# DarylFernandes99/custom-yolo-implmentation

Measured on AMD Instinct MI355X. Metric: images/sec (640x640 bf16), higher is better.
Workload: dtype bf16; 1 GPU; preset s (width 32..512, depth 1) 640x640 train step (fwd+DFL/QFL loss+bwd+grad sync+AdamW), COCO-80 synthetic, 32 img/GPU; global_batch=32, parallelism=dp1, hip_graph=True, optimizer_in_graph=True, deterministic_mode=False

## Files before the change

custom-yolo-implmentation_amd/csrc/conv_generic.hip:

```cpp
#include "conv_host.h"

namespace {

template <typename T, int V, bool ACC>
__global__ void k_conv_generic(ConvGeom g, const T* __restrict__ src, const T* __restrict__ wm,
                               const float* __restrict__ bias, T* __restrict__ dst) {
    long total = (long)g.N * g.Hg * g.Wg * g.Cd;
    for (long i = blockIdx.x * (long)blockDim.x + threadIdx.x; i < total; i += (long)gridDim.x * blockDim.x) {
        int cd = (int)(i % g.Cd);
        long q = i / g.Cd;
        int b = (int)(q % g.Wg);
        long t2 = q / g.Wg;
        int a = (int)(t2 % g.Hg);
        long n = t2 / g.Hg;
        float acc = bias ? bias[cd] : 0.f;
        const T* wrow = wm + (long)cd * g.Kpad;
        for (int t = 0; t < g.ntaps; ++t) {
            int hs = a * g.sstride + g.dh[t], ws = b * g.sstride + g.dw[t];
            if (hs < 0 || hs >= g.Hs || ws < 0 || ws >= g.Ws) continue;
            const T* sp = src + ((n * g.Hs + hs) * g.Ws + ws) * (long)g.lds;
            const T* wp = wrow + t * g.Cs;
            for (int c = 0; c < g.Cs; c += V) {
                float xs[V], wv[V];
                load_pack<T, V>(sp + c, xs);
// ... 218 lines not shown
                                               (const T*)src, (const T*)wm, bias, (T*)dst);
            else hipLaunchKernelGGL((k_conv_generic<T, V, false>), dim3(grid_for(total)), dim3(256), 0, st, g,
                                    (const T*)src, (const T*)wm, bias, (T*)dst);
        } else {
            if (accumulate) hipLaunchKernelGGL((k_conv_generic<T, 1, true>), dim3(grid_for(total)), dim3(256), 0, st, g,
                                               (const T*)src, (const T*)wm, bias, (T*)dst);
            else hipLaunchKernelGGL((k_conv_generic<T, 1, false>), dim3(grid_for(total)), dim3(256), 0, st, g,
                                    (const T*)src, (const T*)wm, bias, (T*)dst);
        }
    });
    return YOLO_LAUNCH_CHECK();
}

}

int valu_conv_launch(const ConvGeom& g, const void* src, const void* wm, const float* bias, void* dst, int accumulate, int dtype,
                     hipStream_t st) {
    int rc = launch_generic(g, src, wm, bias, dst, accumulate, dtype, st);
    if (rc == YOLO_OK && accumulate && g.acc2 != nullptr)
        rc = yolo_copy_channels(g.acc2, g.ld2, dst, g.ldd, (long)g.N * g.Hd * g.Wd, g.Cd, 1, dtype, st);
    if (rc == YOLO_OK && g.stats)
        rc = yolo_bn_stats_acc(dst, g.ldd, (long)g.N * g.Hd * g.Wd, g.Cd, dtype, g.stats, st);
    return rc;
}

extern "C" {

int yolo_conv_kpad(int O, int I, int k, int stride, int mode, int cls) {
    int dh[9], dw[9], kh[9], kw[9];
    int nt = conv_taps(mode, k, stride, cls, dh, dw, kh, kw);
    return round_up32(nt * (mode == 0 ? I : O));
}

long yolo_conv_dgrad_wbuf_elems(int O, int I, int k, int stride) {
    if (stride == 1) return (long)I * yolo_conv_kpad(O, I, k, 1, 1, 0);
    long s = 0;
    for (int c = 0; c < 4; ++c) s += (long)I * yolo_conv_kpad(O, I, k, 2, 1, c);
    return s;
}

int yolo_conv_pack_weights(const void* w_oihw, int w_dtype, int O, int I, int k, int stride, int mode, void* out,
                           int out_dtype, hipStream_t st) {
    if (!conv_supported(k, stride)) return YOLO_ERR_ARG;
    int ncls = (mode == 1 && stride == 2) ? 4 : 1;
    long off = 0;
    for (int c = 0; c < ncls; ++c) {
        TapIdx taps;
        int dh[9], dw[9];
        taps.n = conv_taps(mode, k, stride, c, dh, dw, taps.kh, taps.kw);
        int Kpad = round_up32(taps.n * (mode == 0 ? I : O));
        long total = (long)(mode == 0 ? O : I) * Kpad;
#define PACK_LAUNCH(P)                                                                                               \
    YOLO_DISPATCH_T(out_dtype, hipLaunchKernelGGL((k_pack_weights<P, T>), dim3(grid_for(total)), dim3(256), 0, st,   \
                                                  (const P*)w_oihw, O, I, k, mode, taps, (T*)out + off, Kpad))
        switch (w_dtype) {
            case YOLO_F32:  PACK_LAUNCH(float); break;
            case YOLO_BF16: PACK_LAUNCH(bf16_t); break;
            case YOLO_F16:  PACK_LAUNCH(f16_t); break;
            default: return YOLO_ERR_DTYPE;
        }
#undef PACK_LAUNCH
        off += total;
    }
    return YOLO_LAUNCH_CHECK();
}

int yolo_conv_unpack_wgrad(const float* dwp, int O, int I, int k, void* dw_oihw, int dw_dtype, hipStream_t st) {
    int Kpad = round_up32(k * k * I);
    long total = (long)O * I * k * k;
    switch (dw_dtype) {
        case YOLO_F32:  hipLaunchKernelGGL((k_unpack_wgrad<float>), dim3(grid_for(total)), dim3(256), 0, st, dwp, O, I, k, Kpad, (float*)dw_oihw); break;
        case YOLO_BF16: hipLaunchKernelGGL((k_unpack_wgrad<bf16_t>), dim3(grid_for(total)), dim3(256), 0, st, dwp, O, I, k, Kpad, (bf16_t*)dw_oihw); break;
        case YOLO_F16:  hipLaunchKernelGGL((k_unpack_wgrad<f16_t>), dim3(grid_for(total)), dim3(256), 0, st, dwp, O, I, k, Kpad, (f16_t*)dw_oihw); break;
        default: return YOLO_ERR_DTYPE;
    }
    return YOLO_LAUNCH_CHECK();
}

long yolo_conv2d_wgrad_plan(int N, int H, int W, int Cin, int OH, int OW, int Cout, int k, int stride, int dtype) {
    if (!conv_supported(k, stride)) return -1;
    static const long long dummy[2] = {0, 0};
    if (!mfma_wgrad_eligible(Cin, Cout, Cin, Cout, dtype, dummy, dummy)) return 0;
    return mfma_wgrad2_plan(round_up32(k * k * Cin), N, H, W, Cin, OH, OW, Cout, k);
}

static int wgrad_path(const void* x, int ldx, const void* dy, int ldy, int N, int H, int W, int Cin, int OH, int OW,
                      int Cout, int dtype, int algo) {
    if (algo != 1 && mfma_wgrad_eligible(Cin, Cout, ldx, ldy, dtype, x, dy)) {
        const bool big = (long)N * H * W * ldx + (long)(W + 1) * ldx >= (1L << 30) || (long)N * OH * OW * ldy >= (1L << 30);
        return (algo == 3 || big || (long)N * OH * OW == 0) ? 3 : 2;
    }
    return 1;
}

long yolo_conv2d_wgrad_ws_elems(const void* x, int ldx, const void* dy, int ldy, int N, int H, int W, int Cin, int OH,
                                int OW, int Cout, int k, int stride, int dtype, int algo) {
    if (!conv_supported(k, stride)) return 0;
    const int Kpad = round_up32(k * k * Cin);
    if (wgrad_path(x, ldx, dy, ldy, N, H, W, Cin, OH, OW, Cout, dtype, algo) == 2)
        return mfma_wgrad2_ws_elems(Kpad, N, H, W, Cin, OH, OW, Cout, k);
    return (long)Cout * Kpad;
}

int yolo_conv2d_wgrad(const void* x, int ldx, const void* dy, int ldy, float* ws, void* dw_oihw, int dw_dtype, int N,
                      int H, int W, int Cin, int OH, int OW, int Cout, int k, int stride, int dtype, int algo,
                      hipStream_t st) {
    if (!conv_supported(k, stride)) return YOLO_ERR_ARG;
    const int K = k * k * Cin, Kpad = round_up32(K);
    const int path = wgrad_path(x, ldx, dy, ldy, N, H, W, Cin, OH, OW, Cout, dtype, algo);
    if (path == 2)
        return mfma_wgrad2_launch(x, ldx, dy, ldy, ws, dw_oihw, dw_dtype, Kpad, N, H, W, Cin, OH, OW, Cout, k, stride, dtype, st);
    if (algo == 2) return YOLO_ERR_ARG;
    float* dwp = ws;
    int rc = yolo_zero_async(dwp, (size_t)Cout * Kpad * sizeof(float), st);
    if (rc) return rc;
    if (path == 3) {
        rc = mfma_wgrad_launch(x, ldx, dy, ldy, dwp, Kpad, N, H, W, Cin, OH, OW, Cout, k, stride, dtype, st);
    } else if (dtype == YOLO_F32 && f32_wgrad_eligible(x, ldx, dy, ldy, Cin, Cout)) {
        rc = f32_wgrad_launch((const float*)x, ldx, (const float*)dy, ldy, dwp, Kpad, N, H, W, Cin, OH, OW, Cout, k, stride, st);
    } else {
        long nrows = (long)N * OH;
        long elems = (long)Cout * K;
        int gx = (int)((elems + 255) / 256);
        long want_slabs = 4096 / (gx > 0 ? gx : 1);
        if (want_slabs < 1) want_slabs = 1;
        if (want_slabs > nrows) want_slabs = nrows;
        if (want_slabs < 1) want_slabs = 1;
        int rps = (int)((nrows + want_slabs - 1) / want_slabs);
        if (rps < 1) rps = 1;
        int gy = (int)((nrows + rps - 1) / rps);
        if (gy > 0)
            YOLO_DISPATCH_T(dtype, hipLaunchKernelGGL((k_wgrad_generic<T>), dim3(gx, gy), dim3(256), 0, st, (const T*)x, ldx,
                                                      (const T*)dy, ldy, dwp, Kpad, N, H, W, Cin, OH, OW, Cout, k, stride, rps));
        rc = YOLO_LAUNCH_CHECK();
    }
    if (rc) return rc;
    return yolo_conv_unpack_wgrad(dwp, Cout, Cin, k, dw_oihw, dw_dtype, st);
}

}

static dim3 dw_grid(int nrows, int cv) {
    int tpr = cv < 256 ? cv : 256;
    return dim3((unsigned)(nrows < 4096 ? nrows : 4096), (unsigned)ceil_div(cv, tpr));
}

template <bool FLIP>
static int dw_launch(const void* x, int ldx, const float* w, void* y, int ldy, int N, int H, int W, int C, int dtype,
                     int accumulate, hipStream_t st) {
    const int fast = dw16_launch(FLIP, x, ldx, w, y, ldy, N, H, W, C, dtype, accumulate, nullptr, st);
    if (fast >= 0) return fast;
    YOLO_DISPATCH_T(dtype, {
        if (vecok<T>(x, ldx, C) && vecok<T>(y, ldy, C)) {
            constexpr int V = vec_of<T>::N;
            hipLaunchKernelGGL((k_dw3x3<T, V, FLIP>), dw_grid(N * H, C / V), dim3(256), 0, st, (const T*)x, ldx, w, (T*)y,
                               ldy, N, H, W, C, accumulate);
        } else {
            hipLaunchKernelGGL((k_dw3x3<T, 1, FLIP>), dw_grid(N * H, C), dim3(256), 0, st, (const T*)x, ldx, w, (T*)y, ldy,
                               N, H, W, C, accumulate);
        }
    });
    return YOLO_LAUNCH_CHECK();
}

extern "C" {

// ... 80 lines not shown
```

custom-yolo-implmentation_amd/csrc/conv_host.h:

```cpp
#pragma once
#include "common.h"
#include "conv_geom.h"

enum ConvKind {
    CONV_NONE = -1,
    CONV_VALU = 0,
    CONV_GATHER = 1,
    CONV_HALO = 2,
    CONV_RING = 3,
    CONV_ROWS = 4,
    CONV_UP2 = 5
};
struct RingTile { int bm, bn, nst, bk; };
struct ConvChoice {
    int kind;
    int joint;
    int variant;
    int bn;
    RingTile ring;
};
ConvChoice conv_select(const ConvGeom* gs, int n, int cls, int dtype, const void* src, const void* wm, const void* dst, int algo);

ConvTune& conv_tune();
int conv_wide_flag();

static inline bool desc_addressable(long elems) { return elems < (1L << 30); }
static inline bool pixels_addressable(long npix) { return npix < (1L << 31); }

int mfma_conv_addressable(const ConvGeom& g, int dtype, const void* src, const void* wm, const void* dst);

int valu_conv_launch(const ConvGeom& g, const void* src, const void* wm, const float* bias, void* dst, int accumulate, int dtype,
                     hipStream_t st);
int mfma_conv_eligible(const ConvGeom& g, int dtype, const void* src, const void* wm, const void* dst);
int mfma_conv_launch(const ConvGeom& g, int bn, const void* src, const void* wm, const float* bias, void* dst, int accumulate,
                     int dtype, hipStream_t st);
int halo_conv_eligible(const ConvGeom& g);
int halo_conv_launch(const ConvGeom& g, int variant, const void* src, const void* wm, const float* bias, void* dst,
                     int accumulate, int dtype, hipStream_t st);
int ring_conv_eligible(const ConvGeom& g, int dtype, const void* src, const void* wm, const void* dst);
int ring_conv_launch(const ConvGeom* gs, int n, const RingTile& t, const long* wm_off, long wm_elems, const void* src,
                     const void* wm, const float* bias, void* dst, int accumulate, int dtype, hipStream_t st);
int rows_conv_eligible(const ConvGeom& g);
int rows_conv_launch(const ConvGeom& g, int variant, const void* src, const void* wm, const float* bias, void* dst, int accumulate,
                     int dtype, hipStream_t st);
int up2_conv_eligible(const ConvGeom* gs, int dtype);
int up2_conv_launch(const ConvGeom* gs, int variant, const long* wm_off, long wm_elems, const void* src, const void* wm, void* dst,
                    int accumulate, int dtype, hipStream_t st);
int f32_conv_eligible(const ConvGeom& g, const void* src, const void* wm, const void* dst);
int f32_conv_launch(const ConvGeom& g, const float* src, const float* wm, const float* bias, float* dst, int accumulate,
                    hipStream_t st);

int f32_wgrad_eligible(const void* x, int ldx, const void* dy, int ldy, int Cin, int Cout);
int f32_wgrad_launch(const float* x, int ldx, const float* dy, int ldy, float* dwp, int Kpad, int N, int H, int W, int Cin,
                     int OH, int OW, int Cout, int k, int stride, hipStream_t st);
int mfma_wgrad_eligible(int Cin, int Cout, int ldx, int ldy, int dtype, const void* x, const void* dy);
int mfma_wgrad_launch(const void* x, int ldx, const void* dy, int ldy, float* dwp, int Kpad, int N, int H, int W,
                      int Cin, int OH, int OW, int Cout, int k, int stride, int dtype, hipStream_t st);
long mfma_wgrad2_plan(int Kpad, int N, int H, int W, int Cin, int OH, int OW, int Cout, int k);
long mfma_wgrad2_ws_elems(int Kpad, int N, int H, int W, int Cin, int OH, int OW, int Cout, int k);
int mfma_wgrad2_launch(const void* x, int ldx, const void* dy, int ldy, float* part, void* dw_oihw, int dw_dtype, int Kpad,
                       int N, int H, int W, int Cin, int OH, int OW, int Cout, int k, int stride, int dtype, hipStream_t st);

struct DwPlan {
    int cvb, ncy;
    int ncol, ncb;
    int wg;
    int hb, nb, grid;
    int hb_wg, nb_wg, grid_wg;
};
DwPlan dw_plan(int N, int H, int W, int C);
int dw_tune_set(int variant);
bool dw_takes_rows(int N, int H, int W, int C, bool wgrad);
int dw16_launch(bool flip, const void* x, int ldx, const float* w, void* y, int ldy, int N, int H, int W, int C, int dtype,
                int accumulate, float* stats, hipStream_t st, const float* bias = nullptr, int act = 0);
int dw16_wgrad_launch(const void* x, int ldx, const void* dy, int ldy, float* partial, int nslab, int* nrows, int N, int H, int W,
                      int C, int dtype, hipStream_t st);

extern "C" int yolo_bn_stats_acc(const void* y, int ldy, long npix, int C, int dtype, float* acc, hipStream_t st);
extern "C" int yolo_copy_channels(const void* src, int ld_src, void* dst, int ld_dst, long npix, int C, int accumulate, int dtype,
                                  hipStream_t st);

static inline bool conv_supported(int k, int stride) { return (k == 1 && stride == 1) || (k == 3 && (stride == 1 || stride == 2)); }
```

custom-yolo-implmentation_amd/csrc/wgrad_mfma.hip:

```cpp
#include <cstdio>
#include <cstdlib>
#include "conv_host.h"

namespace {

typedef __attribute__((ext_vector_type(4))) float f32x4;
typedef __attribute__((ext_vector_type(8))) __bf16 bf16x8;
typedef __attribute__((ext_vector_type(8))) _Float16 f16x8;
typedef __attribute__((ext_vector_type(4))) short s16x4;
typedef __attribute__((ext_vector_type(8))) short s16x8;
typedef unsigned int u32x4 __attribute__((ext_vector_type(4)));

template <typename T> struct mm;
template <> struct mm<bf16_t> {
    typedef bf16x8 frag;
    static __device__ __forceinline__ f32x4 mma(frag a, frag b, f32x4 c) { return __builtin_amdgcn_mfma_f32_16x16x32_bf16(a, b, c, 0, 0, 0); }
};
template <> struct mm<f16_t> {
    typedef f16x8 frag;
    static __device__ __forceinline__ f32x4 mma(frag a, frag b, f32x4 c) { return __builtin_amdgcn_mfma_f32_16x16x32_f16(a, b, c, 0, 0, 0); }
};

constexpr int ldc_of(int t) { return t * 32 + 16; }
constexpr int PWL = 12;

struct WgArgs {
    int N, H, W, Cin, ldx, OH, OW, Cout, ldy, Kpad;
    int pbh, pbw;
    long npatch, per_slab;
    int cot, cit;
    int xcd;
};

__device__ __forceinline__ int xcd_chunk(int bid, int nwg) {
    int q = nwg >> 3, r = nwg & 7, x = bid & 7;
    return (x < r ? x * (q + 1) : r * (q + 1) + (x - r) * q) + (bid >> 3);
}

template <typename T>
__device__ __forceinline__ typename mm<T>::frag tr_frag(const T* p_lo, const T* p_hi) {
    s16x4 lo = __builtin_amdgcn_ds_read_tr16_b64_v4i16((__attribute__((address_space(3))) s16x4*)p_lo);
    s16x4 hi = __builtin_amdgcn_ds_read_tr16_b64_v4i16((__attribute__((address_space(3))) s16x4*)p_hi);
    s16x8 both = __builtin_shufflevector(lo, hi, 0, 1, 2, 3, 4, 5, 6, 7);
    return __builtin_bit_cast(typename mm<T>::frag, both);
}

template <typename T, int KS, int S, int TCO, int TCI, int PF>
__global__ __launch_bounds__(256) void k_wgrad2(WgArgs a, const T* __restrict__ x, const T* __restrict__ dy,
                                                float* __restrict__ dwp) {
    constexpr int PAD = KS / 2;
    constexpr int PH = 3 * S + KS, PW = 7 * S + KS;
    constexpr int LDY = ldc_of(TCO), LDX = ldc_of(TCI);
    constexpr int SUB = ((PH + 1) / 2) * PWL;
    constexpr int XROWS = S == 1 ? PH * PWL : 4 * SUB;
    constexpr int CPY = TCO * 4, CPX = TCI * 4;
    constexpr int YCH = 32 * CPY, YR = (YCH + 255) / 256;
    constexpr int XCH = PH * PW * CPX;
    constexpr int XR = (XCH + 255) / 256;
    constexpr int NT = KS * KS;
    static_assert(PW <= PWL || S == 2, "X patch wider than its LDS image");
    static_assert(S == 1 || (PW + 1) / 2 <= PWL, "parity plane wider than its LDS image");
    __shared__ __attribute__((aligned(16))) T ys[32 * LDY];
    __shared__ __attribute__((aligned(16))) T xs[XROWS * LDX];

    const int tid = threadIdx.x, lane = tid & 63, wave = tid >> 6;
    const int wc = wave >> 1, wi = wave & 1;
    const int unit = a.xcd ? xcd_chunk(blockIdx.x, gridDim.x) : (int)blockIdx.x, ntile = a.cot * a.cit;
    const int slab = unit / ntile, tile = unit - slab * ntile;
    const int bco = (tile % a.cot) * (32 * TCO), bci = (tile / a.cot) * (32 * TCI);
    long p_begin = (long)slab * a.per_slab, p_end = p_begin + a.per_slab;
    if (p_end > a.npatch) p_end = a.npatch;

    f32x4 acc[NT][TCO][TCI];
#pragma unroll
    for (int t = 0; t < NT; ++t)
#pragma unroll
        for (int i = 0; i < TCO; ++i)
#pragma unroll
            for (int j = 0; j < TCI; ++j) acc[t][i][j] = (f32x4){0.f, 0.f, 0.f, 0.f};

    const int xshift = (a.W + 1) * a.ldx;
    const __amdgpu_buffer_rsrc_t rsx = buf_desc(x - xshift, (a.N * a.H * a.W * a.ldx + xshift) * 2);
    const __amdgpu_buffer_rsrc_t rsy = buf_desc(dy, a.N * a.OH * a.OW * a.ldy * 2);
    int yrow[YR], ycol[YR], yvoff[YR], ylds[YR];
#pragma unroll
    for (int r = 0; r < YR; ++r) {
        const int id = tid + 256 * r;
        const int j = id / CPY, ch = (id - j * CPY) * 8;
        yrow[r] = j >> 3;
        ycol[r] = j & 7;
        yvoff[r] = (id < YCH && bco + ch < a.Cout) ? ((yrow[r] * a.OW + ycol[r]) * a.ldy + bco + ch) * 2 : BUF_OOB;
        ylds[r] = id < YCH ? ((j & 3) + 4 * ((j >> 3) & 1) + 8 * ((j >> 2) & 1) + 16 * (j >> 4)) * LDY + ch : -1;
    }
    int xpr[XR], xpc[XR], xvoff[XR], xlds[XR];
#pragma unroll
    for (int r = 0; r < XR; ++r) {
        const int id = tid + 256 * r;
        const int px = id / CPX, ch = (id - px * CPX) * 8;
        xpr[r] = px / PW;
        xpc[r] = px - xpr[r] * PW;
        xvoff[r] = (id < XCH && bci + ch < a.Cin) ? ((xpr[r] * a.W + xpc[r]) * a.ldx + bci + ch) * 2 : BUF_OOB;
        const int row = S == 1 ? xpr[r] * PWL + xpc[r]
                               : ((xpr[r] & 1) * 2 + (xpc[r] & 1)) * SUB + (xpr[r] >> 1) * PWL + (xpc[r] >> 1);
        xlds[r] = id < XCH ? row * LDX + ch : -1;
    }
    int pn, pbh, pbw;
    {
        const int per_img = a.pbh * a.pbw;
        pn = (int)(p_begin / per_img);
        const int rem = (int)(p_begin - (long)pn * per_img);
        pbh = rem / a.pbw;
        pbw = rem - pbh * a.pbw;
    }
    uint4 ry[PF][YR], rx[PF][XR];
    auto gload = [&](uint4 (&ry_)[YR], uint4 (&rx_)[XR], bool live) {
        const int oh0 = pbh * 4, ow0 = pbw * 8;
        const int ih0 = oh0 * S - PAD, iw0 = ow0 * S - PAD;
        const int ysoff = live ? ((pn * a.OH + oh0) * a.OW + ow0) * a.ldy * 2 : 0;
#pragma unroll
        for (int r = 0; r < YR; ++r) {
            const bool ok = live && oh0 + yrow[r] < a.OH && ow0 + ycol[r] < a.OW;
            const u32x4 v = __builtin_amdgcn_raw_buffer_load_b128(rsy, ok ? yvoff[r] : BUF_OOB, ysoff, 0);
            ry_[r] = make_uint4(v.x, v.y, v.z, v.w);
        }
        const int xsoff = live ? (((pn * a.H + ih0) * a.W + iw0) * a.ldx + xshift) * 2 : 0;
#pragma unroll
        for (int r = 0; r < XR; ++r) {
            const bool ok = live && (unsigned)(ih0 + xpr[r]) < (unsigned)a.H && (unsigned)(iw0 + xpc[r]) < (unsigned)a.W;
            const u32x4 v = __builtin_amdgcn_raw_buffer_load_b128(rsx, ok ? xvoff[r] : BUF_OOB, xsoff, 0);
            rx_[r] = make_uint4(v.x, v.y, v.z, v.w);
        }
        if (++pbw == a.pbw) {
            pbw = 0;
            if (++pbh == a.pbh) { pbh = 0; ++pn; }
        }
    };
    auto lstore = [&](const uint4 (&ry_)[YR], const uint4 (&rx_)[XR]) {
#pragma unroll
        for (int r = 0; r < YR; ++r)
            if (ylds[r] >= 0) *reinterpret_cast<uint4*>(ys + ylds[r]) = ry_[r];
#pragma unroll
        for (int r = 0; r < XR; ++r)
            if (xlds[r] >= 0) *reinterpret_cast<uint4*>(xs + xlds[r]) = rx_[r];
    };

    const int g = lane >> 4, i16 = lane & 15, q = i16 >> 2, c4 = 4 * (i16 & 3);
    const T* ya = ys + (q + 4 * (g & 1) + 16 * (g >> 1)) * LDY + wc * TCO * 16 + c4;
    auto compute = [&]() {
        typename mm<T>::frag fa[TCO];
#pragma unroll
        for (int i = 0; i < TCO; ++i) fa[i] = tr_frag<T>(ya + i * 16, ya + i * 16 + 8 * LDY);
#pragma unroll
        for (int kh = 0; kh < KS; ++kh)
#pragma unroll
            for (int kw = 0; kw < KS; ++kw) {
                const int row = S == 1 ? (g + kh) * PWL + q + kw
                                       : ((kh & 1) * 2 + (kw & 1)) * SUB + (g + (kh >> 1)) * PWL + q + (kw >> 1);
                const T* base = xs + row * LDX + wi * TCI * 16 + c4;
#pragma unroll
                for (int j = 0; j < TCI; ++j) {
                    typename mm<T>::frag fb = tr_frag<T>(base + j * 16, base + j * 16 + 4 * LDX);
#pragma unroll
                    for (int i = 0; i < TCO; ++i) acc[kh * KS + kw][i][j] = mm<T>::mma(fa[i], fb, acc[kh * KS + kw][i][j]);
                }
            }
    };
#pragma unroll
    for (int s2 = 0; s2 < PF; ++s2) gload(ry[s2], rx[s2], p_begin + s2 < p_end);
    for (long pi = p_begin; pi < p_end; pi += PF) {
#pragma unroll
        for (int s2 = 0; s2 < PF; ++s2) {
            if (pi + s2 >= p_end) break;
            __syncthreads();
            lstore(ry[s2], rx[s2]);
            __syncthreads();
            gload(ry[s2], rx[s2], pi + s2 + PF < p_end);
            compute();
        }
    }
    float4* part4 = reinterpret_cast<float4*>(dwp) + ((((long)slab * ntile + tile) * 4 + wave) * (NT * TCO * TCI)) * 64 + lane;
#pragma unroll
    for (int t = 0; t < NT; ++t)
#pragma unroll
        for (int i = 0; i < TCO; ++i)
#pragma unroll
            for (int j = 0; j < TCI; ++j) {
                const f32x4 v = acc[t][i][j];
                part4[((t * TCO + i) * TCI + j) * 64] = make_float4(v[0], v[1], v[2], v[3]);
            }
}

template <typename TO, int SL>
__global__ __launch_bounds__(256) void k_wgrad_reduce(const float* __restrict__ part, int nslab, int Cout, int Cin, int NT,
                                                      int tco, int tci, int cot, long groups, TO* __restrict__ dw) {
    constexpr int EL = 256 / SL;
    __shared__ float4 red[SL][EL + 1];
    const int el = threadIdx.x % EL, sl = threadIdx.x / EL;
    const long gi = (long)blockIdx.x * EL + el;
    float4 a = make_float4(0.f, 0.f, 0.f, 0.f);
    if (gi < groups) {
        const float4* p = reinterpret_cast<const float4*>(part) + gi;
#pragma unroll 4
        for (int s2 = sl; s2 < nslab; s2 += SL) {
            const float4 v = p[s2 * groups];
            a.x += v.x; a.y += v.y; a.z += v.z; a.w += v.w;
        }
    }
    if (SL > 1) {
        red[sl][el] = a;
        __syncthreads();
        if (sl != 0) return;
#pragma unroll
        for (int s2 = 1; s2 < SL; ++s2) {
            const float4 v = red[s2][el];
            a.x += v.x; a.y += v.y; a.z += v.z; a.w += v.w;
        }
    }
    if (gi < groups) {
        const int lane = (int)(gi & 63);
        long rest = gi >> 6;
        const int j = (int)(rest % tci); rest /= tci;
        const int i = (int)(rest % tco); rest /= tco;
        const int t = (int)(rest % NT); rest /= NT;
        const int wave = (int)(rest & 3);
        const int tile = (int)(rest >> 2);
        const int co = (tile % cot) * (32 * tco) + ((wave >> 1) * tco + i) * 16 + (lane >> 4) * 4;
        const int ci = (tile / cot) * (32 * tci) + ((wave & 1) * tci + j) * 16 + (lane & 15);
        if (ci < Cin) {
            TO* o = dw + ((long)co * Cin + ci) * NT + t;
            const long rs = (long)Cin * NT;
            if (co < Cout) o[0] = (TO)a.x;
            if (co + 1 < Cout) o[rs] = (TO)a.y;
            if (co + 2 < Cout) o[2 * rs] = (TO)a.z;
            if (co + 3 < Cout) o[3 * rs] = (TO)a.w;
        }
    }
}

struct WgPlan { int to, ti, cot, cit, nslab, pf; long per_slab; };

template <typename TO>
void launch_reduce(const float* part, const WgPlan& p, int Cout, int Cin, int NT, void* dw, hipStream_t st) {
    const long groups = (long)p.cot * p.cit * 4 * NT * p.to * p.ti * 64;
    if (p.nslab >= 32)
        hipLaunchKernelGGL((k_wgrad_reduce<TO, 8>), dim3((unsigned)((groups + 31) / 32)), dim3(256), 0, st, part, p.nslab, Cout, Cin, NT, p.to, p.ti, p.cot, groups, (TO*)dw);
    else if (p.nslab >= 4)
        hipLaunchKernelGGL((k_wgrad_reduce<TO, 4>), dim3((unsigned)((groups + 63) / 64)), dim3(256), 0, st, part, p.nslab, Cout, Cin, NT, p.to, p.ti, p.cot, groups, (TO*)dw);
    else
        hipLaunchKernelGGL((k_wgrad_reduce<TO, 1>), dim3((unsigned)((groups + 255) / 256)), dim3(256), 0, st, part, p.nslab, Cout, Cin, NT, p.to, p.ti, p.cot, groups, (TO*)dw);
}



struct WgTune { int to, ti, blocks, min_per; long all_blocks; int pf; };
WgTune& wg_tune() {
    static WgTune t = [] {
        WgTune v{0, 0, 0, 0, 0, 0};
        if (const char* e = getenv("YOLO_WG_TUNE")) sscanf(e, "%d,%d,%d,%d", &v.to, &v.ti, &v.blocks, &v.min_per);
        if (const char* e2 = getenv("YOLO_WG_BLOCKS")) v.all_blocks = atol(e2);
        if (const char* e3 = getenv("YOLO_WG_PF")) v.pf = atoi(e3);
        return v;
    }();
    return t;
}

WgPlan make_plan(const WgArgs& a, int k) {
    WgPlan p;
    if (k == 1) {
        p.to = a.Cout > 96 ? 4 : a.Cout > 64 ? 3 : a.Cout > 32 ? 2 : 1;
        p.ti = a.Cin > 96 ? 4 : a.Cin > 64 ? 3 : a.Cin > 32 ? 2 : 1;
    } else {
        p.to = a.Cout > 32 ? 2 : 1;
        p.ti = a.Cin > 64 ? 2 : 1;
    }
    const int cot0 = (a.Cout + 32 * p.to - 1) / (32 * p.to), cit0 = (a.Cin + 32 * p.ti - 1) / (32 * p.ti);
    const long data_bytes = ((long)a.N * a.H * a.W * a.Cin + (long)a.N * a.OH * a.OW * a.Cout) * 2;
    long want_blocks;
    const WgTune& tu = wg_tune();
    if (tu.all_blocks > 0) {
        want_blocks = tu.all_blocks;
    } else if (k == 1) {
        if (p.to * p.ti == 1) want_blocks = 2048;
        else want_blocks = (cot0 * cit0 == 1 && data_bytes < (150L << 20)) ? 256 : 512;
    } else {
        want_blocks = p.ti == 1 ? 512 : 256;
    }
    {
        static const double scale = [] { const char* e = getenv("YOLO_WG_SCALE"); return e ? atof(e) : 0.5; }();
        if (scale > 0.0 && tu.all_blocks <= 0 && tu.blocks <= 0) {
            const long tile_bytes = (long)k * k * (32 * p.to) * (32 * p.ti) * 4;
            long cap = (long)(scale * (double)data_bytes / (double)tile_bytes);
            static const long floor_wg = [] { const char* e = getenv("YOLO_WG_FLOOR"); return e ? atol(e) : 128L; }();
            if (cap < floor_wg) cap = floor_wg;
            if (want_blocks > cap) want_blocks = cap;
        }
    }
    long min_per = 2;
    if (tu.to > 0 && (k == 1 || tu.to <= 2)) p.to = tu.to;
    if (tu.ti > 0 && (k == 1 || tu.ti <= 2)) p.ti = tu.ti;
    if (tu.blocks > 0) want_blocks = tu.blocks;
    if (tu.min_per > 0) min_per = tu.min_per;
    p.cot = (a.Cout + 32 * p.to - 1) / (32 * p.to);
    p.cit = (a.Cin + 32 * p.ti - 1) / (32 * p.ti);
    long want = want_blocks / ((long)p.cot * p.cit);
    if (want > a.npatch / min_per) want = a.npatch / min_per;
    if (want < 1) want = 1;
    p.per_slab = (a.npatch + want - 1) / want;
    p.nslab = (int)((a.npatch + p.per_slab - 1) / p.per_slab);
    p.pf = 1;
    if (tu.pf == 1 || tu.pf == 4) p.pf = tu.pf;
    return p;
}

template <typename T, int KS, int S, int TCO, int TCI>
void launch(const WgArgs& a, const WgPlan& p, const void* x, const void* dy, float* part, hipStream_t st) {
    WgArgs b = a;
    b.per_slab = p.per_slab;
    b.cot = p.cot; b.cit = p.cit;
    static const int xcd = [] { const char* e = getenv("YOLO_WG_XCD"); return e ? atoi(e) : 1; }();
    b.xcd = xcd;
    const dim3 grid((unsigned)(p.cot * p.cit * p.nslab));
    if (p.pf == 4)
        hipLaunchKernelGGL((k_wgrad2<T, KS, S, TCO, TCI, 4>), grid, dim3(256), 0, st, b, (const T*)x, (const T*)dy, part);
    else
        hipLaunchKernelGGL((k_wgrad2<T, KS, S, TCO, TCI, 1>), grid, dim3(256), 0, st, b, (const T*)x, (const T*)dy, part);
}

template <typename T, int KS, int S>
void launch_tiles(const WgArgs& a, const WgPlan& p, const void* x, const void* dy, float* part, hipStream_t st) {
#define WG_CASE(TO_, TI_) if (p.to == TO_ && p.ti == TI_) return launch<T, KS, S, TO_, TI_>(a, p, x, dy, part, st)
    if constexpr (KS == 1) {
        WG_CASE(1, 1); WG_CASE(1, 2); WG_CASE(1, 3); WG_CASE(1, 4);
        WG_CASE(2, 1); WG_CASE(2, 2); WG_CASE(2, 3); WG_CASE(2, 4);
        WG_CASE(3, 1); WG_CASE(3, 2); WG_CASE(3, 3); WG_CASE(3, 4);
        WG_CASE(4, 1); WG_CASE(4, 2); WG_CASE(4, 3); WG_CASE(4, 4);
    } else {
        WG_CASE(1, 1); WG_CASE(1, 2); WG_CASE(2, 1); WG_CASE(2, 2);
    }
#undef WG_CASE
}

template <typename T>
int launch_ks(const WgArgs& a, const WgPlan& p, int k, int stride, const void* x, const void* dy, float* part,
              hipStream_t st) {
    if (k == 1 && stride == 1) launch_tiles<T, 1, 1>(a, p, x, dy, part, st);
    else if (k == 3 && stride == 1) launch_tiles<T, 3, 1>(a, p, x, dy, part, st);
    else if (k == 3 && stride == 2) launch_tiles<T, 3, 2>(a, p, x, dy, part, st);
    else return YOLO_ERR_ARG;
    return YOLO_LAUNCH_CHECK();
}

WgArgs make_args(int ldx, int ldy, int Kpad, int N, int H, int W, int Cin, int OH, int OW, int Cout) {
    WgArgs a;
    a.N = N; a.H = H; a.W = W; a.Cin = Cin; a.ldx = ldx; a.OH = OH; a.OW = OW; a.Cout = Cout; a.ldy = ldy; a.Kpad = Kpad;
    a.pbh = (OH + 3) / 4; a.pbw = (OW + 7) / 8;
    a.npatch = (long)N * a.pbh * a.pbw;
    a.per_slab = 0;
    return a;
}

}

extern "C" int yolo_wgrad_tune_set(int to, int ti, int blocks, int min_per) {
    WgTune& t = wg_tune();
    t.to = to; t.ti = ti; t.blocks = blocks; t.min_per = min_per;
    return YOLO_OK;
}

extern "C" int yolo_wgrad_tune_pf(int pf) {
    if (pf != 0 && pf != 1 && pf != 4) return YOLO_ERR_ARG;
    wg_tune().pf = pf;
    return YOLO_OK;
}

long mfma_wgrad2_ws_elems(int Kpad, int N, int H, int W, int Cin, int OH, int OW, int Cout, int k) {
    WgArgs a = make_args(0, 0, Kpad, N, H, W, Cin, OH, OW, Cout);
    if (a.npatch == 0) return (long)Cout * Kpad;
    const WgPlan p = make_plan(a, k);
    return (long)p.nslab * p.cot * p.cit * k * k * (32L * p.to) * (32L * p.ti);
}

long mfma_wgrad2_plan(int Kpad, int N, int H, int W, int Cin, int OH, int OW, int Cout, int k) {
    WgArgs a = make_args(0, 0, Kpad, N, H, W, Cin, OH, OW, Cout);
    if (a.npatch == 0) return 0;
    const WgPlan p = make_plan(a, k);
    return p.pf * 10000000L + p.to * 1000000L + p.ti * 100000L + p.nslab;
}

int mfma_wgrad2_launch(const void* x, int ldx, const void* dy, int ldy, float* part, void* dw_oihw, int dw_dtype, int Kpad,
                       int N, int H, int W, int Cin, int OH, int OW, int Cout, int k, int stride, int dtype, hipStream_t st) {
    WgArgs a = make_args(ldx, ldy, Kpad, N, H, W, Cin, OH, OW, Cout);
    if (a.npatch == 0) return YOLO_ERR_ARG;
    const WgPlan p = make_plan(a, k);
    int rc;
    if (dtype == YOLO_BF16) rc = launch_ks<bf16_t>(a, p, k, stride, x, dy, part, st);
    else if (dtype == YOLO_F16) rc = launch_ks<f16_t>(a, p, k, stride, x, dy, part, st);
    else return YOLO_ERR_DTYPE;
    if (rc) return rc;
    if (dw_dtype == YOLO_F32) launch_reduce<float>(part, p, Cout, Cin, k * k, dw_oihw, st);
    else if (dw_dtype == YOLO_BF16) launch_reduce<bf16_t>(part, p, Cout, Cin, k * k, dw_oihw, st);
    else if (dw_dtype == YOLO_F16) launch_reduce<f16_t>(part, p, Cout, Cin, k * k, dw_oihw, st);
    else return YOLO_ERR_DTYPE;
    return YOLO_LAUNCH_CHECK();
}
```

include/yolo_hip.h:

```cpp
#ifndef YOLO_HIP_H
#define YOLO_HIP_H
#include <stddef.h>
#include <stdint.h>

#ifdef __cplusplus
extern "C" {
#endif

#ifndef __HIP__
typedef struct ihipStream_t* hipStream_t;
#endif

#define YOLO_F32 0
#define YOLO_BF16 1
#define YOLO_F16 2
#define YOLO_ERR_ARG 1001
#define YOLO_ERR_DTYPE 1002
#define YOLO_ACT_IDENTITY 0
#define YOLO_ACT_SILU 1

long yolo_abi_hash(void);

int yolo_memset0(void* p, size_t bytes, hipStream_t st);
int yolo_ncm_to_nhwc(const void* src, int src_dtype, long sn, long sc, long off, void* dst, int dst_dtype, int ld, int N, int C, int HW, hipStream_t st);
int yolo_nhwc_to_ncm(const void* src, int src_dtype, int ld, void* dst, int dst_dtype, long sn, long sc, long off, int N, int C, int HW, hipStream_t st);
int yolo_head_group(int pack, int n, void* const* branches, const int* lds, const int* Cs, const int* HWs, const int* c_offs, const int* m_offs, void* preds, int cp, int M, int N, int dtype, hipStream_t st);
int yolo_copy_channels(const void* src, int ld_src, void* dst, int ld_dst, long npix, int C, int accumulate, int dtype, hipStream_t st);
int yolo_scale_inplace(void* x, long n, int dtype, const float* scale_dev, hipStream_t st);
int yolo_add_n(const void* s0, int ld0, const void* s1, int ld1, const void* s2, int ld2, const void* s3, int ld3, int nsrc, void* dst, int ld_dst, long npix, int C, int dtype, hipStream_t st);

int yolo_conv_kpad(int O, int I, int k, int stride, int mode, int cls);
long yolo_conv_dgrad_wbuf_elems(int O, int I, int k, int stride);
int yolo_conv_pack_weights(const void* w_oihw, int w_dtype, int O, int I, int k, int stride, int mode, void* out, int out_dtype, hipStream_t st);
int yolo_conv_unpack_wgrad(const float* dwp, int O, int I, int k, void* dw_oihw, int dw_dtype, hipStream_t st);
int yolo_pack_job_bytes();
int yolo_pack_job_count(int stride, int mode);
long yolo_pack_job_fill(void* jobs_host, const void* w, int w_dtype, void* out, int out_elem_bytes, int O, int I, int k, int stride, int mode, long start);
long yolo_pack_jobs_finalize(void* jobs_host, int njobs);
int yolo_pack_batched(const void* jobs_dev, int njobs, long nchunks, int out_dtype, hipStream_t st);
int yolo_adamw_job_bytes();
int yolo_adamw_job_fill(void* jobs_host, int index, void* p, int p_dtype, const void* g, int g_dtype, float* m, float* v, long n);
long yolo_adamw_jobs_finalize(void* jobs_host, int njobs);
int yolo_adamw_jobs_set_grads(void* jobs_host, int njobs, const void* const* grads);
int yolo_adamw_step(const void* jobs_dev, int njobs, long nchunks, const double* hyper, float* step, const float* grad_scale, const float* found_inf, hipStream_t st);
int yolo_adamw_job_set_ema(void* jobs_host, int index, float* ema, double* ema_ctl);
int yolo_ema_lerp(const void* jobs_dev, int njobs, long nchunks, const double* ema_ctl, const float* skip_flag, hipStream_t st);
int yolo_adamw_amp_step(const void* jobs_dev, int njobs, long nchunks, const double* hyper, float* step, float* amp_state, int* growth_tracker, float growth_factor, float backoff_factor, int growth_interval, hipStream_t st);
int yolo_grad_sqnorm(const void* jobs_dev, int njobs, long nchunks, float* partials, float* found_inf, hipStream_t st);
int yolo_grad_clip_finalize(const float* partials, long nparts, float* clip_state, const float* grad_scale, hipStream_t st);
int yolo_adamw_clip_step(const void* jobs_dev, int njobs, long nchunks, const double* hyper, float* step, const float* grad_scale, const float* found_inf, const float* clip_state, hipStream_t st);
int yolo_amp_update_scale(float* amp_state, int* growth_tracker, float growth_factor, float backoff_factor, int growth_interval, hipStream_t st);
int yolo_sgd_step(const void* jobs_dev, int njobs, long nchunks, const double* hyper, float* step, const float* grad_scale, const float* found_inf, const float* clip_state, hipStream_t st);
int yolo_sgd_amp_step(const void* jobs_dev, int njobs, long nchunks, const double* hyper, float* step, float* amp_state, int* growth_tracker, float growth_factor, float backoff_factor, int growth_interval, hipStream_t st);
int yolo_copy_job_bytes();
int yolo_copy_job_fill(void* jobs_host, int index, const void* src, int src_dtype, void* dst, int dst_dtype, long n);
long yolo_copy_jobs_finalize(void* jobs_host, int njobs);
int yolo_multi_copy(const void* jobs_dev, int njobs, long nchunks, float scale, hipStream_t st);
int yolo_conv2d_fwd(const void* x, int ldx, const void* wp, const float* bias, void* y, int ldy, float* stats_acc, int N, int H, int W, int Cin, int OH, int OW, int Cout, int k, int stride, int dtype, int algo, hipStream_t st);
int yolo_conv2d_fwd_act(const void* x, int ldx, const void* wp, const float* bias, const void* res, int ldr, void* y, int ldy, int N, int H, int W, int Cin, int OH, int OW, int Cout, int k, int stride, int act, int dtype, hipStream_t st);
int yolo_conv2d_dgrad(const void* dy, int lddy, const void* wb, void* dx, int lddx, int N, int H, int W, int Cin, int OH, int OW, int Cout, int k, int stride, int accumulate, int dtype, int algo, hipStream_t st);
int yolo_conv2d_dgrad_acc2(const void* dy, int lddy, const void* wb, void* dx, int lddx, const void* acc2, int ld2, int N, int H, int W, int Cin, int OH, int OW, int Cout, int k, int stride, int dtype, int algo, hipStream_t st);
long yolo_conv2d_wgrad_ws_elems(const void* x, int ldx, const void* dy, int ldy, int N, int H, int W, int Cin, int OH, int OW, int Cout, int k, int stride, int dtype, int algo);
int yolo_conv2d_wgrad(const void* x, int ldx, const void* dy, int ldy, float* ws, void* dw_oihw, int dw_dtype, int N, int H, int W, int Cin, int OH, int OW, int Cout, int k, int stride, int dtype, int algo, hipStream_t st);
int yolo_conv_tune_set(int bn, int tap_inner, int halo, int dma, int ring, int bm, int nst, int bk);
int yolo_wgrad_tune_set(int to, int ti, int blocks, int min_per);
int yolo_wgrad_tune_pf(int pf);
int yolo_conv_wide_set(int on);
int yolo_conv2d_plan(int N, int H, int W, int Cin, int OH, int OW, int Cout, int k, int stride, int mode, int cls, int dtype);
long yolo_conv2d_wgrad_plan(int N, int H, int W, int Cin, int OH, int OW, int Cout, int k, int stride, int dtype);
int yolo_stem_im2col(const void* img, int img_dtype, void* col, int col_dtype, int N, int H, int W, int OH, int OW, hipStream_t st);
int yolo_stem_pack_weights(const void* w, int w_dtype, int Cout, void* out, int out_dtype, hipStream_t st);
int yolo_stem_unpack_wgrad(const float* dw32, int Cout, void* dw, int dw_dtype, hipStream_t st);
int yolo_stem_conv_eligible(int img_dtype, int dtype, int Cout);
int yolo_stem_conv_fwd(const float* img, const void* wp, void* y, int ldy, float* stats, int N, int H, int W, int OH, int OW, int Cout, const float* bias, int act, int dtype, hipStream_t st);
int yolo_stem_wgrad_slabs();
int yolo_stem_wgrad(const float* img, const void* dy, int ldy, float* partial, void* dw, int dw_dtype, int N, int H, int W, int OH, int OW, int Cout, int dtype, hipStream_t st);
int yolo_dwconv3x3_fwd(const void* x, int ldx, const float* w, void* y, int ldy, int N, int H, int W, int C, int dtype, hipStream_t st);
int yolo_dwconv3x3_fwd_stats(const void* x, int ldx, const float* w, void* y, int ldy, float* stats, int N, int H, int W, int C, int dtype, hipStream_t st);
int yolo_dwconv3x3_fwd_act(const void* x, int ldx, const float* w, const float* bias, void* y, int ldy, int N, int H, int W, int C, int act, int dtype, hipStream_t st);
int yolo_dwconv3x3_dgrad(const void* dy, int lddy, const float* w, void* dx, int lddx, int N, int H, int W, int C, int accumulate, int dtype, hipStream_t st);
int yolo_dw_wgrad_nslab(int N, int H);
int yolo_dwconv3x3_wgrad(const void* x, int ldx, const void* dy, int ldy, float* dw, float* partial, int N, int H, int W, int C, int dtype, hipStream_t st);
int yolo_dw_tune_set(int variant);
int yolo_dw_plan(int N, int H, int W, int C, int field);

int yolo_reduce_nblk(long npix, int C);
int yolo_bn_stats(const void* y, int ldy, long npix, int C, int dtype, float* partial, int nblk, hipStream_t st);
int yolo_bn_finalize(const float* partial, int nblk, long count, int C, const void* gamma, const void* beta, void* running_mean, void* running_var, float momentum, float eps, float* mean, float* invstd, float* scale, float* shift, int pdtype, int bdtype, hipStream_t st);
int yolo_bn_eval_coeffs(const void* gamma, const void* beta, const void* running_mean, const void* running_var, float eps, int C, float* scale, float* shift, int pdtype, int bdtype, hipStream_t st);
int yolo_sum_finalize(const float* partial, int nblk, int C, float* out, hipStream_t st);
int yolo_bn_act_fwd(const void* y, int ldy, const float* scale, const float* shift, const void* res, int ldres, void* out, int ldout, long npix, int C, int act, int dtype, hipStream_t st);
int yolo_bn_act_bwd_reduce(const void* dout, int ldd, const void* y, int ldy, const float* scale, const float* shift, const float* mean, const float* invstd, long npix, int C, int act, int dtype, float* partial, int nblk, hipStream_t st);
int yolo_bn_bwd_finalize(const float* partial, int nblk, long count, int C, const void* gamma, const float* mean, const float* invstd, void* dgamma, void* dbeta, float* coef, int pdtype, hipStream_t st);
int yolo_bn_act_bwd_apply(const void* dout, int ldd, const void* y, int ldy, const float* scale, const float* shift, const float* mean, const float* invstd, const float* coef, void* dy, int lddy, long npix, int C, int act, int dtype, hipStream_t st);
int yolo_bn_acc_elems(int C);
int yolo_bn_stats_acc(const void* y, int ldy, long npix, int C, int dtype, float* acc, hipStream_t st);
int yolo_bn_finalize_acc(const float* acc, long count, int C, const void* gamma, const void* beta, void* running_mean, void* running_var, float momentum, float eps, float* mean, float* invstd, float* scale, float* shift, int pdtype, int bdtype, hipStream_t st);
int yolo_bn_act_fwd_train(const void* y, int ldy, const float* acc, long count, const void* gamma, const void* beta, void* running_mean, void* running_var, float momentum, float eps, float* mean, float* invstd, float* scale, float* shift, const void* res, int ldres, void* out, int ldout, long npix, int C, int act, int dtype, int pdtype, int bdtype, hipStream_t st);
int yolo_bn_bwd_reduce_acc(const void* dout, int ldd, const void* y, int ldy, const float* scale, const float* shift, long npix, int C, int act, int dtype, float* acc, hipStream_t st);
int yolo_bn_act_bwd_apply_train(const void* dout, int ldd, const void* y, int ldy, const float* scale, const float* shift, const void* gamma, const float* mean, const float* invstd, const float* acc, long count, void* dgamma, void* dbeta, void* dy, int lddy, long npix, int C, int act, int dtype, int pdtype, hipStream_t st);

int yolo_maxpool5_fwd(const void* x, int ldx, void* out, int ldo, uint8_t* idx, int N, int H, int W, int C, int dtype, hipStream_t st);
int yolo_maxpool5_bwd(const void* dout, int ldd, const uint8_t* idx, void* dx, int ldx, int N, int H, int W, int C, int accumulate, int dtype, hipStream_t st);
int yolo_upsample2x_fwd(const void* x, int ldx, void* out, int ldo, int N, int H, int W, int C, int dtype, hipStream_t st);
int yolo_upsample2x_bwd(const void* dout, int ldd, void* dx, int ldx, int N, int H, int W, int C, int accumulate, int dtype, hipStream_t st);

size_t yolo_attn_stash_bytes(int N, int T_, int heads, int dtype);
size_t yolo_attn_workspace_bytes(int N, int T_, int heads, int dtype);
size_t yolo_attn_stash_bytes_for(int N, int T, int heads, int dk, int dh, int dtype);
size_t yolo_attn_workspace_bytes_for(int N, int T, int heads, int dk, int dh, int dtype);
int yolo_attn_fwd(const void* qkv, int ldq, void* o, int ldo, void* vp, int ldv, void* stash, void* ws, int N, int T_, int heads, int dk, int dh, float scale, int dtype, hipStream_t st);
int yolo_attn_fwd_nograd(const void* qkv, int ldq, void* o, int ldo, void* vp, int ldv, int N, int T_, int heads, int dk, int dh, float scale, int dtype, hipStream_t st);
int yolo_attn_bwd(const void* qkv, int ldq, const void* o, int ldo, const void* d_o, int lddo, const void* d_vp, int lddv, const void* stash, void* ws, void* dqkv, int lddq, int N, int T_, int heads, int dk, int dh, float scale, int dtype, hipStream_t st);

size_t yolo_loss_workspace_bytes(int N, int A, int G);
int yolo_loss_dfl_qfl(const void* preds, const void* anchors, const void* strides, int dtype, int N, int nc, int A, const float* gt, const int* gt_off, const int* gt_img, int G, float lambda_dfl, float lambda_cls, void* dpreds, float* out, void* workspace, const float* grad_scale, hipStream_t st);

size_t yolo_loss_tal_workspace_bytes(int N, int A, int G);
int yolo_loss_tal(const void* preds, const void* anchors, const void* strides, int dtype, int N, int nc, int A, const float* gt, const int* gt_off, const int* gt_img, int G, int topk, float alpha, float beta, float lambda_box, float lambda_cls, float lambda_dfl, void* dpreds, float* out, void* workspace, const float* grad_scale, hipStream_t st);

int yolo_bbox_iou(const float* box1, const float* box2, int M, float* iou, const float* g, float* db1, float* db2, hipStream_t st);
int yolo_quality_focal_loss(const float* pred, const float* target, int M, int C, float beta, float* out, const float* g, float* dpred, float* dtarget, hipStream_t st);
int yolo_distribution_focal_loss(const float* pred_dist, const float* target_val, int M, int C, float* out, const float* g, float* dpred, float* dtarget, hipStream_t st);

int yolo_head_decode(const void* preds, const void* anchors, const void* strides, void* y, int N, int nc, int A, int dtype, hipStream_t st);
int yolo_dfl_expect(const void* x, void* y, int B, int A, int dtype, hipStream_t st);
int yolo_nms_capacity(int M, int nc, int multi_label);
size_t yolo_nms_workspace_bytes(int bs, int M, int nc, int multi_label);
int yolo_nms(const void* y, int dtype, int bs, int nc, int M, float conf_thres, float iou_thres, const int* classes, int n_classes, int agnostic, int multi_label, int max_det, float* out, int* out_count, int* status, void* workspace, hipStream_t st);

size_t yolo_val_workspace_bytes(int N, int M, int top_k);
int yolo_val_select(const void* y, int dtype, int N, int nc, int M, float conf, int top_k, float* out, int* out_count, void* workspace, hipStream_t st);
int yolo_val_match(const float* pred, const int* count, int N, int top_k, const float* gt, const int* gt_off, double iou_thr, int nc, int skip_empty_gt, long long* counters, int* status, hipStream_t st);

int yolo_prep_image_bytes();
int yolo_prep_image_fill(void* table_host, int index, long off, int H, int W, int flip, int o0, int o1, int o2, int o3, float brightness, float contrast, float saturation, float hue);
int yolo_image_prep(const void* src, const void* table_dev, int N, int S, int jitter, void* stage, float* means, void* out, int out_dtype, float m0, float m1, float m2, float s0, float s1, float s2, hipStream_t st);
int yolo_mosaic_tile_bytes();
int yolo_mosaic_tile_fill(void* table_host, int image, int tile, long off, int H, int W, int flip, int tw, int th, int x0, int y0, int cx, int cy);
int yolo_image_prep_mosaic(const void* src, const void* tiles_dev, const void* table_dev, int N, int S, int fill, int jitter, void* stage, float* means, void* out, int out_dtype, float m0, float m1, float m2, float s0, float s1, float s2, hipStream_t st);
int yolo_affine_bytes();
int yolo_affine_fill(void* table_host, int index, float a00, float a01, float b0, float a10, float a11, float b1);
int yolo_image_prep_affine(const void* src, const void* tiles_dev, const void* table_dev, const void* affine_dev, int N, int S, int fill, int jitter, void* stage, void* stage2, float* means, void* out, int out_dtype, float m0, float m1, float m2, float s0, float s1, float s2, hipStream_t st);

int yolo_selftest_tr16(const void* tile_in, void* out, hipStream_t st);
int yolo_selftest_glds(const void* in128x16, void* out64x16, hipStream_t st);
int yolo_selftest_dma_vs_xlane(const void* pattern4k, int blocks, int iters, int spam, void* errors, void* sink, hipStream_t st);
int yolo_selftest_dma_order(const void* src, long src_bytes, int blocks, int kind, void* errors2, hipStream_t st);
int yolo_selftest_ring_vs_xlane(const void* src, int steps, int blocks, int spam, void* errors, void* sink, hipStream_t st);
int yolo_selftest_permlane16(const void* in64, void* out128, hipStream_t st);
int yolo_selftest_grid_barrier(void* counters, int blocks, int rounds, int tree, int* timed_out, hipStream_t st);

// ... 5 lines not shown
```

Baseline: 3076 images/s.

## Add two K-group wgrad kernel splitting patches across 512-thread blocks with LDS fold

Adds a KG=2 variant of the MFMA weight-gradient kernel. Two 256-thread groups in one block each take alternate patches of the slab, each with its own LDS staging buffer, and their accumulators are folded through LDS before one partial is written. The planner picks this variant by default when slabs stay long enough, and halves the slab count, so fewer partials need to be written and reduced. The cost is doubled LDS per block, a fold phase, and possibly lower occupancy.

New measurement: 3094 images/s, median of 6. Within noise of the previous version (+0.6%).

```diff
diff --git a/custom-yolo-implmentation_amd/csrc/conv_generic.hip b/custom-yolo-implmentation_amd/csrc/conv_generic.hip
--- a/custom-yolo-implmentation_amd/csrc/conv_generic.hip
+++ b/custom-yolo-implmentation_amd/csrc/conv_generic.hip
@@ -324,6 +324,13 @@
     static const long long dummy[2] = {0, 0};
     if (!mfma_wgrad_eligible(Cin, Cout, Cin, Cout, dtype, dummy, dummy)) return 0;
     return mfma_wgrad2_plan(round_up32(k * k * Cin), N, H, W, Cin, OH, OW, Cout, k);
+}
+
+int yolo_conv2d_wgrad_kgroups(int N, int H, int W, int Cin, int OH, int OW, int Cout, int k, int stride, int dtype) {
+    if (!conv_supported(k, stride)) return -1;
+    static const long long dummy[2] = {0, 0};
+    if (!mfma_wgrad_eligible(Cin, Cout, Cin, Cout, dtype, dummy, dummy)) return 0;
+    return mfma_wgrad2_kgroups(round_up32(k * k * Cin), N, H, W, Cin, OH, OW, Cout, k);
 }
 
 static int wgrad_path(const void* x, int ldx, const void* dy, int ldy, int N, int H, int W, int Cin, int OH, int OW,
diff --git a/custom-yolo-implmentation_amd/csrc/conv_host.h b/custom-yolo-implmentation_amd/csrc/conv_host.h
--- a/custom-yolo-implmentation_amd/csrc/conv_host.h
+++ b/custom-yolo-implmentation_amd/csrc/conv_host.h
@@ -57,6 +57,7 @@
 int mfma_wgrad_launch(const void* x, int ldx, const void* dy, int ldy, float* dwp, int Kpad, int N, int H, int W,
                       int Cin, int OH, int OW, int Cout, int k, int stride, int dtype, hipStream_t st);
 long mfma_wgrad2_plan(int Kpad, int N, int H, int W, int Cin, int OH, int OW, int Cout, int k);
+int mfma_wgrad2_kgroups(int Kpad, int N, int H, int W, int Cin, int OH, int OW, int Cout, int k);
 long mfma_wgrad2_ws_elems(int Kpad, int N, int H, int W, int Cin, int OH, int OW, int Cout, int k);
 int mfma_wgrad2_launch(const void* x, int ldx, const void* dy, int ldy, float* part, void* dw_oihw, int dw_dtype, int Kpad,
                        int N, int H, int W, int Cin, int OH, int OW, int Cout, int k, int stride, int dtype, hipStream_t st);
diff --git a/custom-yolo-implmentation_amd/csrc/wgrad_mfma.hip b/custom-yolo-implmentation_amd/csrc/wgrad_mfma.hip
--- a/custom-yolo-implmentation_amd/csrc/wgrad_mfma.hip
+++ b/custom-yolo-implmentation_amd/csrc/wgrad_mfma.hip
@@ -45,8 +45,8 @@
     return __builtin_bit_cast(typename mm<T>::frag, both);
 }
 
-template <typename T, int KS, int S, int TCO, int TCI, int PF>
-__global__ __launch_bounds__(256) void k_wgrad2(WgArgs a, const T* __restrict__ x, const T* __restrict__ dy,
+template <typename T, int KS, int S, int TCO, int TCI, int PF, int KG>
+__global__ __launch_bounds__(256 * KG) void k_wgrad2(WgArgs a, const T* __restrict__ x, const T* __restrict__ dy,
                                                 float* __restrict__ dwp) {
     constexpr int PAD = KS / 2;
     constexpr int PH = 3 * S + KS, PW = 7 * S + KS;
@@ -60,10 +60,14 @@
     constexpr int NT = KS * KS;
     static_assert(PW <= PWL || S == 2, "X patch wider than its LDS image");
     static_assert(S == 1 || (PW + 1) / 2 <= PWL, "parity plane wider than its LDS image");
-    __shared__ __attribute__((aligned(16))) T ys[32 * LDY];
-    __shared__ __attribute__((aligned(16))) T xs[XROWS * LDX];
-
-    const int tid = threadIdx.x, lane = tid & 63, wave = tid >> 6;
+    static_assert(KG == 1 || (KG == 2 && PF == 1), "two K-groups: one patch in flight per group");
+    constexpr int STAGE = 32 * LDY + XROWS * LDX;
+    __shared__ __attribute__((aligned(16))) T stage[KG * STAGE];
+
+    const int grp = KG == 1 ? 0 : __builtin_amdgcn_readfirstlane((int)threadIdx.x >> 8);
+    const int tid = threadIdx.x & 255, lane = tid & 63, wave = tid >> 6;
+    T* const ys = stage + grp * STAGE;
+    T* const xs = ys + 32 * LDY;
     const int wc = wave >> 1, wi = wave & 1;
     const int unit = a.xcd ? xcd_chunk(blockIdx.x, gridDim.x) : (int)blockIdx.x, ntile = a.cot * a.cit;
     const int slab = unit / ntile, tile = unit - slab * ntile;
@@ -107,8 +111,8 @@
     int pn, pbh, pbw;
     {
         const int per_img = a.pbh * a.pbw;
-        pn = (int)(p_begin / per_img);
-        const int rem = (int)(p_begin - (long)pn * per_img);
+        pn = (int)((p_begin + grp) / per_img);
+        const int rem = (int)(p_begin + grp - (long)pn * per_img);
         pbh = rem / a.pbw;
         pbw = rem - pbh * a.pbw;
     }
@@ -130,10 +134,12 @@
             const u32x4 v = __builtin_amdgcn_raw_buffer_load_b128(rsx, ok ? xvoff[r] : BUF_OOB, xsoff, 0);
             rx_[r] = make_uint4(v.x, v.y, v.z, v.w);
         }
-        if (++pbw == a.pbw) {
-            pbw = 0;
-            if (++pbh == a.pbh) { pbh = 0; ++pn; }
-        }
+#pragma unroll
+        for (int s2 = 0; s2 < KG; ++s2)
+            if (++pbw == a.pbw) {
+                pbw = 0;
+                if (++pbh == a.pbh) { pbh = 0; ++pn; }
+            }
     };
     auto lstore = [&](const uint4 (&ry_)[YR], const uint4 (&rx_)[XR]) {
 #pragma unroll
@@ -165,18 +171,55 @@
                 }
             }
     };
-#pragma unroll
-    for (int s2 = 0; s2 < PF; ++s2) gload(ry[s2], rx[s2], p_begin + s2 < p_end);
-    for (long pi = p_begin; pi < p_end; pi += PF) {
-#pragma unroll
-        for (int s2 = 0; s2 < PF; ++s2) {
-            if (pi + s2 >= p_end) break;
+    if constexpr (KG == 1) {
+#pragma unroll
+        for (int s2 = 0; s2 < PF; ++s2) gload(ry[s2], rx[s2], p_begin + s2 < p_end);
+        for (long pi = p_begin; pi < p_end; pi += PF) {
+#pragma unroll
+            for (int s2 = 0; s2 < PF; ++s2) {
+                if (pi + s2 >= p_end) break;
+                __syncthreads();
+                lstore(ry[s2], rx[s2]);
+                __syncthreads();
+                gload(ry[s2], rx[s2], pi + s2 + PF < p_end);
+                compute();
+            }
+        }
+    } else {
+        const int len = (int)(p_end - p_begin);
+        gload(ry[0], rx[0], grp < len);
+        for (int t = 0; t < len; t += 2) {
+            const bool mine = t + grp < len;
             __syncthreads();
-            lstore(ry[s2], rx[s2]);
+            if (mine) lstore(ry[0], rx[0]);
             __syncthreads();
-            gload(ry[s2], rx[s2], pi + s2 + PF < p_end);
-            compute();
-        }
+            gload(ry[0], rx[0], t + grp + 2 < len);
+            if (mine) compute();
+        }
+        constexpr int NBLK = NT * TCO * TCI;
+        constexpr int FIT = (int)(KG * STAGE * sizeof(T) / 4096), NB = FIT < NBLK ? FIT : NBLK;
+        static_assert(NB >= 1, "staging LDS smaller than one accumulator block");
+        float4* fold = reinterpret_cast<float4*>(stage) + tid;
+#pragma unroll
+        for (int b0 = 0; b0 < NBLK; b0 += NB) {
+            __syncthreads();
+            if (grp == 1) {
+#pragma unroll
+                for (int b = b0; b < b0 + NB && b < NBLK; ++b) {
+                    const f32x4 v = acc[b / (TCO * TCI)][b / TCI % TCO][b % TCI];
+                    fold[(b - b0) * 256] = make_float4(v[0], v[1], v[2], v[3]);
+                }
+            }
+            __syncthreads();
+            if (grp == 0) {
+#pragma unroll
+                for (int b = b0; b < b0 + NB && b < NBLK; ++b) {
+                    const float4 v = fold[(b - b0) * 256];
+                    acc[b / (TCO * TCI)][b / TCI % TCO][b % TCI] += (f32x4){v.x, v.y, v.z, v.w};
+                }
+            }
+        }
+        if (grp != 0) return;
     }
     float4* part4 = reinterpret_cast<float4*>(dwp) + ((((long)slab * ntile + tile) * 4 + wave) * (NT * TCO * TCI)) * 64 + lane;
 #pragma unroll
@@ -237,7 +280,7 @@
     }
 }
 
-struct WgPlan { int to, ti, cot, cit, nslab, pf; long per_slab; };
+struct WgPlan { int to, ti, cot, cit, nslab, pf, kg; long per_slab; };
 
 template <typename TO>
 void launch_reduce(const float* part, const WgPlan& p, int Cout, int Cin, int NT, void* dw, hipStream_t st) {
@@ -252,13 +295,15 @@
 
 
 
-struct WgTune { int to, ti, blocks, min_per; long all_blocks; int pf; };
+struct WgTune { int to, ti, blocks, min_per; long all_blocks; int pf, kg; };
 WgTune& wg_tune() {
     static WgTune t = [] {
-        WgTune v{0, 0, 0, 0, 0, 0};
+        WgTune v{0, 0, 0, 0, 0, 0, 0};
         if (const char* e = getenv("YOLO_WG_TUNE")) sscanf(e, "%d,%d,%d,%d", &v.to, &v.ti, &v.blocks, &v.min_per);
         if (const char* e2 = getenv("YOLO_WG_BLOCKS")) v.all_blocks = atol(e2);
         if (const char* e3 = getenv("YOLO_WG_PF")) v.pf = atoi(e3);
+        if (const char* e4 = getenv("YOLO_WG_KG")) v.kg = atoi(e4);
+        if (v.kg < 0 || v.kg > 3) v.kg = 0;
         return v;
     }();
     return t;
@@ -285,6 +330,7 @@
     } else {
         want_blocks = p.ti == 1 ? 512 : 256;
     }
+    const long base_blocks = want_blocks;
     {
         static const double scale = [] { const char* e = getenv("YOLO_WG_SCALE"); return e ? atof(e) : 0.5; }();
         if (scale > 0.0 && tu.all_blocks <= 0 && tu.blocks <= 0) {
@@ -302,13 +348,27 @@
     if (tu.min_per > 0) min_per = tu.min_per;
     p.cot = (a.Cout + 32 * p.to - 1) / (32 * p.to);
     p.cit = (a.Cin + 32 * p.ti - 1) / (32 * p.ti);
-    long want = want_blocks / ((long)p.cot * p.cit);
-    if (want > a.npatch / min_per) want = a.npatch / min_per;
-    if (want < 1) want = 1;
-    p.per_slab = (a.npatch + want - 1) / want;
-    p.nslab = (int)((a.npatch + p.per_slab - 1) / p.per_slab);
     p.pf = 1;
     if (tu.pf == 1 || tu.pf == 4) p.pf = tu.pf;
+    auto slabs = [&](long blocks) {
+        long want = blocks / ((long)p.cot * p.cit);
+        if (want > a.npatch / min_per) want = a.npatch / min_per;
+        if (want < 1) want = 1;
+        p.per_slab = (a.npatch + want - 1) / want;
+        p.nslab = (int)((a.npatch + p.per_slab - 1) / p.per_slab);
+    };
+    const bool free_count = tu.blocks <= 0 && tu.all_blocks <= 0;
+    p.kg = 1;
+    slabs(want_blocks);
+    if (p.pf != 4 && tu.kg >= 2) {
+        p.kg = 2;
+        if (tu.kg == 2 && free_count) slabs(want_blocks / 2);
+    } else if (p.pf != 4 && tu.kg == 0 && free_count) {
+        const WgPlan one = p;
+        p.kg = 2;
+        slabs(want_blocks < base_blocks / 2 ? want_blocks : base_blocks / 2);
+        if (p.per_slab < 2 * min_per) p = one;
+    }
     return p;
 }
 
@@ -321,9 +381,11 @@
     b.xcd = xcd;
     const dim3 grid((unsigned)(p.cot * p.cit * p.nslab));
     if (p.pf == 4)
-        hipLaunchKernelGGL((k_wgrad2<T, KS, S, TCO, TCI, 4>), grid, dim3(256), 0, st, b, (const T*)x, (const T*)dy, part);
+        hipLaunchKernelGGL((k_wgrad2<T, KS, S, TCO, TCI, 4, 1>), grid, dim3(256), 0, st, b, (const T*)x, (const T*)dy, part);
+    else if (p.kg == 2)
+        hipLaunchKernelGGL((k_wgrad2<T, KS, S, TCO, TCI, 1, 2>), grid, dim3(512), 0, st, b, (const T*)x, (const T*)dy, part);
     else
-        hipLaunchKernelGGL((k_wgrad2<T, KS, S, TCO, TCI, 1>), grid, dim3(256), 0, st, b, (const T*)x, (const T*)dy, part);
+        hipLaunchKernelGGL((k_wgrad2<T, KS, S, TCO, TCI, 1, 1>), grid, dim3(256), 0, st, b, (const T*)x, (const T*)dy, part);
 }
 
 template <typename T, int KS, int S>
@@ -373,6 +435,12 @@
     return YOLO_OK;
 }
 
+extern "C" int yolo_wgrad_tune_kg(int kg) {
+    if (kg < 0 || kg > 3) return YOLO_ERR_ARG;
+    wg_tune().kg = kg;
+    return YOLO_OK;
+}
+
 long mfma_wgrad2_ws_elems(int Kpad, int N, int H, int W, int Cin, int OH, int OW, int Cout, int k) {
     WgArgs a = make_args(0, 0, Kpad, N, H, W, Cin, OH, OW, Cout);
     if (a.npatch == 0) return (long)Cout * Kpad;
@@ -385,6 +453,12 @@
     if (a.npatch == 0) return 0;
     const WgPlan p = make_plan(a, k);
     return p.pf * 10000000L + p.to * 1000000L + p.ti * 100000L + p.nslab;
+}
+
+int mfma_wgrad2_kgroups(int Kpad, int N, int H, int W, int Cin, int OH, int OW, int Cout, int k) {
+    WgArgs a = make_args(0, 0, Kpad, N, H, W, Cin, OH, OW, Cout);
+    if (a.npatch == 0) return 0;
+    return make_plan(a, k).kg;
 }
 
 int mfma_wgrad2_launch(const void* x, int ldx, const void* dy, int ldy, float* part, void* dw_oihw, int dw_dtype, int Kpad,
diff --git a/include/yolo_hip.h b/include/yolo_hip.h
--- a/include/yolo_hip.h
+++ b/include/yolo_hip.h
@@ -65,9 +65,11 @@
 int yolo_conv_tune_set(int bn, int tap_inner, int halo, int dma, int ring, int bm, int nst, int bk);
 int yolo_wgrad_tune_set(int to, int ti, int blocks, int min_per);
 int yolo_wgrad_tune_pf(int pf);
+int yolo_wgrad_tune_kg(int kg);
 int yolo_conv_wide_set(int on);
 int yolo_conv2d_plan(int N, int H, int W, int Cin, int OH, int OW, int Cout, int k, int stride, int mode, int cls, int dtype);
 long yolo_conv2d_wgrad_plan(int N, int H, int W, int Cin, int OH, int OW, int Cout, int k, int stride, int dtype);
+int yolo_conv2d_wgrad_kgroups(int N, int H, int W, int Cin, int OH, int OW, int Cout, int k, int stride, int dtype);
 int yolo_stem_im2col(const void* img, int img_dtype, void* col, int col_dtype, int N, int H, int W, int OH, int OW, hipStream_t st);
 int yolo_stem_pack_weights(const void* w, int w_dtype, int Cout, void* out, int out_dtype, hipStream_t st);
 int yolo_stem_unpack_wgrad(const float* dw32, int Cout, void* dw, int dw_dtype, hipStream_t st);
```
